# LPMP/BDD

Measured on AMD Instinct MI355X. Metric: parallel-MMA iterations/sec, 10.5M BDD nodes, 1 GPU (+ achieved HBM GB/s in roofline), higher is better.
Workload: dtype f32

## Files before the change

### bdd_amd/capi.py

```python
from __future__ import annotations

import ctypes as C
import os
import subprocess

_HERE = os.path.dirname(os.path.abspath(__file__))
LIB_PATH = os.path.abspath(os.environ["BDDMMA_LIB"]) if os.environ.get("BDDMMA_LIB") else os.path.join(_HERE, "csrc", "libbdd_mma_hip.so")

OK = 0
F32, F64 = 0, 1
K_FORWARD_MM, K_BACKWARD_MM, K_FINISH_DELTA, K_OTHER, K_COUNT = 0, 1, 2, 3, 4


class Options(C.Structure):
    _fields_ = [("pack_width", C.c_uint32), ("wide_pack_width", C.c_uint32), ("deterministic", C.c_uint32),
                ("vars_per_bin", C.c_uint32), ("stage_cap", C.c_uint32), ("waves_per_block", C.c_uint32),
                ("keep_bdd_order", C.c_uint32), ("resident_sweeps", C.c_uint32), ("exchange_by_variable", C.c_uint32),
                ("variant_flags", C.c_uint32), ("pack_fill", C.c_uint32), ("pack_stagger", C.c_uint32)]


class LbfgsParams(C.Structure):
    _fields_ = [("history_size", C.c_int32), ("init_step_size", C.c_double), ("req_rel_lb_increase", C.c_double),
                ("step_size_decrease_factor", C.c_double), ("step_size_increase_factor", C.c_double)]

# ... 58 lines not shown
    "bddmma_min_marginals": (_I, [_V, _I, _V, _V, _V, _I]),
    "bddmma_min_marginal_diff": (_I, [_V, _V, _I]),
    "bddmma_bdds_solution": (_I, [_V, _I, _V, _I]),
    "bddmma_net_solver_costs": (_I, [_V, _V, _I]),
    "bddmma_make_dual_feasible": (_I, [_V, _V, _I]),
    "bddmma_gradient_step": (_I, [_V, _V, _D, _I]),
    "bddmma_lbfgs_create": (_I, [C.POINTER(_V), _V, C.POINTER(LbfgsParams)]),
    "bddmma_lbfgs_destroy": (None, [_V]),
    "bddmma_lbfgs_iteration": (_I, [_V]),
    "bddmma_lbfgs_update_costs": (_I, [_V, _V, _U64, _V, _U64, _I, _I]),
    "bddmma_lbfgs_flush": (_I, [_V]),
    "bddmma_lbfgs_get_state": (_I, [_V, C.POINTER(LbfgsState)]),
    "bddmma_perturb_primal_costs": (_I, [_V, _V, _D, C.c_uint32, C.c_uint32, C.POINTER(C.c_uint32), _V, _V, _V]),
    "bddmma_run_solver": (_I, [_V, _V, _U64, _D, _D, _D, _I, C.POINTER(RunResult)]),
    "bddmma_run_solver_host_loop": (_I, [_V, _V, _U64, _D, _D, _D, _I, C.POINTER(RunResult)]),
    "bddmma_incremental_mm_agreement_rounding": (_I, [_V, _V, _D, _D, _U64, _U64, C.c_uint32, _I, _V, C.POINTER(_I)]),
    "bddmma_save": (_I, [_V, C.c_char_p]),
    "bddmma_load": (_I, [C.POINTER(_V), _I, C.c_char_p]),
    "bddmma_synchronize": (_I, [_V]),
    "bddmma_set_profiling": (_I, [_V, _I]),
    "bddmma_get_profile": (_I, [_V, C.POINTER(Profile)]),
    "bddmma_time_iterations": (_I, [_V, _D, _U64, C.POINTER(_D)]),
    "bddmma_time_kernel": (_I, [_V, _I, _U64, C.POINTER(_D)]),
    "bddmma_device_bytes": (_U64, [_V]),
    "bddmma_device_allocated_bytes": (_U64, [_V]),
    "bddmma_layout_create": (_I, [C.POINTER(_V), _V, _V, _U64, C.POINTER(Options)]),
    "bddmma_layout_create_for_chip": (_I, [C.POINTER(_V), _V, _V, _U64, C.POINTER(Options), _I, C.c_uint32, C.c_uint32]),
    "bddmma_layout_destroy": (None, [_V]),
    "bddmma_layout_size": (_U64, [_V, _I]),
    "bddmma_layout_copy": (_I, [_V, _I, _V]),
    "bddmma_layout_res2_records": (_I, [_V, _I, _V, _V, _V]),
    "bddmma_layout_stream_records": (_I, [_V, _I, _V, _V, _V]),
    "bddmma_layout_layer_records": (_I, [_V, _I, _V, _V, _V]),
    "bddmma_layout_seg_exchange": (_I, [_V, _I, _I, _V, _V, _V, _V]),
}

_I64P, _U64P = C.POINTER(C.c_int64), C.POINTER(C.c_uint64)
ILP_SIGNATURES = {
    "bddilp_last_error": (C.c_char_p, []),
    "bddilp_parse_lp": (_I, [C.c_char_p, C.POINTER(_V)]),
    "bddilp_parse_opb": (_I, [C.c_char_p, C.POINTER(_V)]),
    "bddilp_parse": (_I, [C.c_char_p, C.POINTER(_V)]),
    "bddilp_destroy": (None, [_V]),
    "bddilp_nr_variables": (_U64, [_V]),
    "bddilp_nr_constraints": (_U64, [_V]),
    "bddilp_variable_name": (C.c_char_p, [_V, _U64]),
    "bddilp_objective": (_I, [_V, _V, C.POINTER(_D)]),
    "bddilp_constraint_size": (_U64, [_V, _U64]),
    "bddilp_constraint": (_I, [_V, _U64, _V, _V, C.POINTER(_I), C.POINTER(C.c_int64)]),
    "bddilp_constraint_name": (C.c_char_p, [_V, _U64]),
    "bddilp_normalize": (_I, [_V]),
    "bddilp_to_bdds": (_I, [_V, _I, _U64, C.POINTER(_V)]),
    "bddilp_bdds_create": (_I, [C.POINTER(_V)]),
    "bddilp_bdds_add_row": (_I, [_V, _V, _V, _U64, _I, C.c_int64, C.POINTER(_I)]),
    "bddilp_bdds_split": (_I, [_V, _U64, _U64, _I, _U64P, _U64P]),
    "bddilp_bdds_destroy": (None, [_V]),
    "bddilp_bdds_nr_bdds": (_U64, [_V]),
    "bddilp_bdds_nr_instructions": (_U64, [_V]),
    "bddilp_bdds_nr_variables": (_U64, [_V]),
    "bddilp_bdds_instructions": (_V, [_V]),
    "bddilp_bdds_delimiters": (_V, [_V]),
    "bddilp_write_bdd_lp": (_I, [_V, _V, _U64, _V, _U64, C.c_char_p]),
    "bddilp_export_graphviz": (_I, [_V, _V, _U64, _U64, C.c_char_p]),
    "bddilp_random_set_cover": (_I, [_U64, _U64, _U64, _U64, _V, _V]),
}

# ... 35 lines not shown
```

### bdd_amd/csrc/capi.cpp

```cpp
#include <chrono>
#include <cmath>
#include <cstdio>
#include <cstdlib>
#include <cstring>
#include <limits>
#include <new>
#include <string>
#include <vector>

#include "../../include/bdd_mma.h"
#include "layout.hpp"
#include "solver.hpp"

using namespace bddmma;

struct bddmma_lbfgs;
extern "C" int bddmma_lbfgs_iteration(bddmma_lbfgs* l);
extern "C" int bddmma_lbfgs_update_costs(bddmma_lbfgs* l, const void* lo, uint64_t n_lo, const void* hi, uint64_t n_hi, int elem_precision,
                                         int on_device);

namespace {
thread_local std::string g_err;

template <typename F>
// ... 779 lines not shown
    if (!l || !info || (real_size != 4 && real_size != 8) || threads <= 0) return BDDMMA_ERR_INVALID_ARGUMENT;
    SegExchange S;
    build_seg_exchange(l->L, (uint32_t)threads, (uint32_t)real_size, S);
    info[0] = S.ok ? 1u : 0u; info[1] = (uint32_t)S.bin.size(); info[2] = (uint32_t)S.perm.size(); info[3] = (uint32_t)S.thr.size();
    info[4] = S.max_entries; info[5] = S.max_slots; info[6] = S.max_groups;
    if (bin && !S.bin.empty()) std::memcpy(bin, S.bin.data(), S.bin.size() * sizeof(uint32_t));
    if (perm && !S.perm.empty()) std::memcpy(perm, S.perm.data(), S.perm.size() * sizeof(uint16_t));
    if (thr && !S.thr.empty()) std::memcpy(thr, S.thr.data(), S.thr.size() * sizeof(uint32_t));
    return BDDMMA_OK;
}

int bddmma_layout_stream_records(const bddmma_layout* l, int real_size, uint32_t* info, uint32_t* words, uint32_t* rec_off)
{
    if (!l || !info || (real_size != 4 && real_size != 8)) return BDDMMA_ERR_INVALID_ARGUMENT;
    StreamRecords R;
    build_stream_records(l->L, (uint32_t)real_size, R);
    info[0] = R.ok ? 1u : 0u; info[1] = (uint32_t)R.rec.size();
    if (words && !R.rec.empty()) std::memcpy(words, R.rec.data(), R.rec.size() * sizeof(uint32_t));
    if (rec_off && !R.rec_off.empty()) std::memcpy(rec_off, R.rec_off.data(), R.rec_off.size() * sizeof(uint32_t));
    return BDDMMA_OK;
}

int bddmma_layout_layer_records(const bddmma_layout* l, int real_size, uint32_t* info, uint32_t* words, uint32_t* rec_off)
{
    if (!l || !info || (real_size != 4 && real_size != 8)) return BDDMMA_ERR_INVALID_ARGUMENT;
    LayerRecords R;
    build_layer_records(l->L, (uint32_t)real_size, R);
    info[0] = R.ok ? 1u : 0u; info[1] = (uint32_t)R.rec.size();
    if (words && !R.rec.empty()) std::memcpy(words, R.rec.data(), R.rec.size() * sizeof(uint32_t));
    if (rec_off && !R.rec_off.empty()) std::memcpy(rec_off, R.rec_off.data(), R.rec_off.size() * sizeof(uint32_t));
    return BDDMMA_OK;
}

}
```

### bdd_amd/csrc/kernels/narrow3.hpp

```cpp
#pragma once

namespace bddmma {

constexpr int N3_W = 128;
template <typename REAL>
__device__ __forceinline__ void lds_ld2(REAL& a, REAL& b, const unsigned char* lds, uint32_t off)
{
    const REAL* p = reinterpret_cast<const REAL*>(lds + off);
    a = p[0];
    b = p[1];
}

template <typename REAL, bool NT>
__device__ __forceinline__ void pot_pair_load(typename Pair<REAL>::type& v, rsrc_t rh, uint32_t voff, uint32_t soff)
{
    constexpr int AUX = NT ? 2 : BDDMMA_LD_POT_AUX;
    if constexpr (sizeof(REAL) == 4) v = __builtin_bit_cast(float2, __builtin_amdgcn_raw_buffer_load_b64(rh, voff, soff, AUX));
    else v = __builtin_bit_cast(double2, __builtin_amdgcn_raw_buffer_load_b128(rh, voff, soff, AUX));
}

__device__ __forceinline__ void pot_store(float v, rsrc_t rh, uint32_t voff, uint32_t soff, uint32_t ) { hop_store(v, rh, voff, soff); }
__device__ __forceinline__ void pot_store(double v, rsrc_t rh, uint32_t voff, uint32_t soff, uint32_t nt)
{
    if (nt) hop_store<2>(v, rh, voff, soff);
    else hop_store<>(v, rh, voff, soff);
}

template <typename REAL>
__device__ __forceinline__ void pot_store_layer(REAL a, REAL b, bool two, rsrc_t rh, uint32_t off_a, uint32_t soff, uint32_t nt)
{
    using P2 = typename Pair<REAL>::type;
    const uint32_t off2 = two ? off_a : (uint32_t)LREC_NO_STORE, off1 = two ? (uint32_t)LREC_NO_STORE : off_a;
    P2 v;
    v.x = a;
    v.y = b;
    if constexpr (sizeof(REAL) == 4) {
        using u2 = decltype(__builtin_amdgcn_raw_buffer_load_b64(rh, 0, 0, 0));
        __builtin_amdgcn_raw_buffer_store_b64(__builtin_bit_cast(u2, v), rh, off2, soff, BDDMMA_ST_FT_AUX_F32);
        pot_store(a, rh, off1, soff, nt);
    } else {
        using u4 = decltype(__builtin_amdgcn_raw_buffer_load_b128(rh, 0, 0, 0));
        const u4 data = __builtin_bit_cast(u4, v);
        if (nt) __builtin_amdgcn_raw_buffer_store_b128(data, rh, off2, soff, 2);
// ... 28 lines not shown
    const uint32_t quad = block_to_pack(block_id, n_quads, pk.xcd_chunk);
    BDDMMA_EXIT_IF(quad >= n_quads, d)
    const uint32_t p = quad * WPB + wave;
    const bool has_pack = p < pk.n_packs;
    const bool hdr = pk.hdr_pack != nullptr;
    const uint32_t* const hp = hdr ? pk.hdr_pack + 8 * (size_t)(has_pack ? p : 0) : nullptr;
    const uint32_t q0 = !has_pack ? 0 : (hdr ? hp[4] : pk.pack_hop_ptr[p]);
    const uint32_t q1 = !has_pack ? 0 : (hdr ? q0 + (hp[5] & 0xFFFFu) : pk.pack_hop_ptr[p + 1]);
    const uint32_t rbase = has_pack ? lrec_off[p] : 0;
    const uint32_t c0_h = hdr ? pk.hdr_quad[4 * (size_t)quad] : 0, cnt_h = hdr ? pk.hdr_quad[4 * (size_t)quad + 1] : 0;
    BDDMMA_STAMP(p, 0);
    const REAL INF = inf_v<REAL>();
    const uint32_t slot_first = !has_pack ? 0 : (hdr ? hp[0] : pk.hop_node_off[q0]), l0 = !has_pack ? 0 : (hdr ? hp[2] : pk.hop_layer_off[q0]);
    NarrowRs<REAL> rs(d);
    rs.rebase_layers(d, l0);
    uint32_t ent[STAGE_ITERS], esl[STAGE_ITERS];
    if (hdr) stage_load_tables<REAL, WPB, (NT ? 2 : BDDMMA_LD_TAB_AUX)>(ent, esl, rs, c0_h, cnt_h, tid);
    REAL* const Tp = d.T + slot_first;
    REAL* const Fp = d.F + slot_first;
    const REAL* const lohi_p = d.lohi + 2 * (size_t)l0;
    const rsrc_t rr = make_rsrc(lrec, lrec_words);
    HopWindow hw{sOffN_[wave], sOffL_[wave], sOffR_[wave], q0, q1, slot_first, l0};
    constexpr int D = LA;
    uint32_t o[2 * D + 3];
    uint32_t lb[D + 2];
    u4v rc[2 * D + 1];
    P2 tr[D + 1];
    P2 Lr[D + 1];
#pragma unroll
    for (int i = 0; i < 2 * D + 3; ++i) o[i] = 0;
#pragma unroll
    for (int i = 0; i < D + 2; ++i) lb[i] = 0;
    auto ldrec = [&](uint32_t h) { return __builtin_amdgcn_raw_buffer_load_b128(rr, (uint32_t)lane * 16u, (rbase + h * 64u) * 16u, 0); };
    const uint32_t sink = (W + 2 * (uint32_t)lane) * S;
    if (has_pack) {
        hw.fill(pk, q0, lane);
#pragma unroll
        for (int i = 0; i < 2 * D + 3; ++i) o[i] = hw.node_off(q0 + i);
#pragma unroll
        for (int i = 0; i < D + 2; ++i) lb[i] = hw.layer_off(q0 + i);
#pragma unroll
        for (int r = 0; r < 2; ++r) {
            const uint32_t j = lane + 64 * r;
            lds_st<REAL>(sFw, j * S, (j < o[1] - o[0]) ? REAL(0) : INF);
        }
#pragma unroll
        for (int b = 0; b < 2; ++b) {
            lds_st<REAL>(sTw, b * BUF + sink, REAL(0));
            lds_st<REAL>(sTw, b * BUF + sink + S, INF);
        }
#pragma unroll
        for (int i = 0; i < 2 * D; ++i) rc[i] = ldrec((uint32_t)i);
        {
            P2 t1;
            pot_pair_load<REAL, NT>(t1, hop_rsrc(Tp, o[1], o[2] - o[1]), 2u * (uint32_t)lane * S, o[1] * S);
#pragma unroll
            for (int i = 0; i < D; ++i) pot_pair_load<REAL, NT>(tr[i], hop_rsrc(Tp, o[i + 2], o[i + 3] - o[i + 2]), 2u * (uint32_t)lane * S, o[i + 2] * S);
            if (2u * (uint32_t)lane < o[2] - o[1]) lds_st<P2>(sTw, 2u * (uint32_t)lane * S, t1);
        }
#pragma unroll
        for (int i = 0; i < D; ++i) hop_load(Lr[i], rs.lohi, (uint32_t)lane * (uint32_t)sizeof(P2), lb[i] * (uint32_t)sizeof(P2));
        wave_sync();
    } else {
#pragma unroll
        for (int i = 0; i < 2 * D; ++i) rc[i] = u4v{0u, 0u, 0u, 0u};
    }
    uint32_t cur = 0;
    uint32_t q = q0;
    const uint32_t g0 = (has_pack && !hdr) ? pk.pack_group_ptr[p] : 0;
    const uint32_t ng = !has_pack ? 0 : (hdr ? 1u : pk.pack_group_ptr[p + 1] - g0);
    const uint32_t r0 = hdr ? 0 : pk.quad_round_ptr[quad];
    const uint32_t n_rounds = hdr ? 1u : pk.quad_round_ptr[quad + 1] - r0;
    const uint32_t db = (uint32_t)wave * pk.stage_cap * (uint32_t)sizeof(P2);
    for (uint32_t k = 0; k < n_rounds; ++k) {
    uint32_t gl0 = 0, cnt = 0, qe = q1;
    if (hdr) {
        cnt = cnt_h;
        stage_load_pairs<REAL, WPB>(sD, ent, esl, rs, cnt, tid);
        qe = has_pack ? q1 : q;
    } else {
        const uint32_t c0 = pk.cs_ptr[r0 + k];
        cnt = pk.cs_ptr[r0 + k + 1] - c0;
        stage_load<REAL, WPB, (NT ? 2 : BDDMMA_LD_TAB_AUX)>(sD, ent, esl, rs, c0, cnt, tid);
        if (k < ng) {
            gl0 = pk.grp_layer_off[g0 + k] - l0;
            qe = pk.grp_hop_end[g0 + k];
        } else {
            qe = q;
        }
    }
    if (WPB > 1) __syncthreads(); else wave_sync();
    BDDMMA_STAMP(p, 1);
    auto hop = [&]() {
        if (q + 2 * D + 3 >= hw.base + HOP_WIN && hw.base + HOP_WIN <= q1) hw.fill(pk, q, lane);
        const uint32_t nb = o[0];
        const uint32_t n3 = o[3] - o[2];
        const uint32_t fc = cur * BUF, fn = (cur ^ 1u) * BUF;
        const uint32_t stg = db + (lb[0] - gl0 + (uint32_t)lane) * (uint32_t)sizeof(P2);
        rc[2 * D] = ldrec(q - q0 + 2 * D);
#ifndef BDDMMA_EXP_NO_HOP_LOADS
        pot_pair_load<REAL, NT>(tr[D], hop_rsrc(Tp, o[D + 2], o[D + 3] - o[D + 2]), 2u * (uint32_t)lane * S, o[D + 2] * S);
        hop_load(Lr[D], rs.lohi, (uint32_t)lane * (uint32_t)sizeof(P2), lb[D] * (uint32_t)sizeof(P2));
#endif
        const u4v ra = rc[0];
        const P2 c = Lr[0];
        const uint32_t flags = ra[2] >> 16;
        REAL fa, fb;
        lds_ld2(fa, fb, sFw, fc + (ra[2] & 0xFFFFu));
        const REAL tla = lds_ld<REAL>(sTw, fc + (ra[0] & 0xFFFFu)), tha = lds_ld<REAL>(sTw, fc + (ra[0] >> 16));
        const REAL tlb = lds_ld<REAL>(sTw, fc + (ra[1] & 0xFFFFu)), thb = lds_ld<REAL>(sTw, fc + (ra[1] >> 16));
        const P2 dd = lds_ld<P2>(dyn_lds, stg);
        const uint32_t o_new = hw.node_off(q + 2 * D + 3);
        const uint32_t l_next = hw.layer_off(q + D + 2);
        if (2u * (uint32_t)lane < n3) lds_st<P2>(sTw, fn + 2u * (uint32_t)lane * S, tr[0]);
        lds_st<P2>(sFw, fn + 2u * (uint32_t)lane * S, P2{INF, INF});
        wave_sync();
        fa = (flags & LREC_REAL) ? fa : INF;
        fb = (flags & LREC_TWO) ? fb : INF;
        const REAL m0 = rmin((fa + c.x) + tla, (fb + c.x) + tlb);
        const REAL m1 = rmin((fa + c.y) + tha, (fb + c.y) + thb);
        const REAL mm = mm_diff1(m0, m1, omega);
        P2 nc;
        nc.x = (c.x + min0(mm)) + dd.x;
        nc.y = (c.y + min0_neg(mm)) + dd.y;
#ifndef BDDMMA_EXP_NO_HOP_STORES
        const rsrc_t rl = hop_rsrc(reinterpret_cast<const P2*>(lohi_p), lb[0], lb[1] - lb[0]);
        hop_store(nc, rl, (uint32_t)lane * (uint32_t)sizeof(P2), lb[0] * (uint32_t)sizeof(P2));
#endif
        if (flags & LREC_REAL) lds_st<REAL>(dyn_lds, stg, mm);
        lds_min(reinterpret_cast<REAL*>(sFw + fn + (ra[0] & 0xFFFFu)), fa + nc.x);
        lds_min(reinterpret_cast<REAL*>(sFw + fn + (ra[0] >> 16)), fa + nc.y);
        lds_min(reinterpret_cast<REAL*>(sFw + fn + (ra[1] & 0xFFFFu)), fb + nc.x);
        lds_min(reinterpret_cast<REAL*>(sFw + fn + (ra[1] >> 16)), fb + nc.y);
#ifndef BDDMMA_EXP_NO_HOP_STORES
        {
            const rsrc_t rf = hop_rsrc(Fp, nb, o[1] - o[0]);
            pot_store_layer<REAL>(fa, fb, (flags & LREC_TWO) != 0, rf, ra[3] & 0xFFFFu, nb * S, pk.nt_potentials);
        }
#endif
        wave_sync();
        cur ^= 1u;
#pragma unroll
        for (int i = 0; i < 2 * D + 2; ++i) o[i] = o[i + 1];
        o[2 * D + 2] = o_new;
#pragma unroll
        for (int i = 0; i < D + 1; ++i) lb[i] = lb[i + 1];
        lb[D + 1] = l_next;
#pragma unroll
// ... 55 lines not shown
    const uint32_t q0 = !has_pack ? 0 : (hdr ? hp[4] : pk.pack_hop_ptr[p]);
    const uint32_t q1 = !has_pack ? 0 : (hdr ? q0 + (hp[5] & 0xFFFFu) : pk.pack_hop_ptr[p + 1]);
    const uint32_t rbase = has_pack ? lrec_off[p] : 0;
    const uint32_t c0_h = hdr ? pk.hdr_quad[4 * (size_t)quad] : 0, cnt_h = hdr ? pk.hdr_quad[4 * (size_t)quad + 1] : 0;
    BDDMMA_STAMP(p, 0);
    const REAL INF = inf_v<REAL>();
    const uint32_t slot_first = !has_pack ? 0 : (hdr ? hp[0] : pk.hop_node_off[q0]), l0 = !has_pack ? 0 : (hdr ? hp[2] : pk.hop_layer_off[q0]);
    NarrowRs<REAL> rs(d);
    rs.rebase_layers(d, l0);
    uint32_t ent[STAGE_ITERS], esl[STAGE_ITERS];
    if (hdr) stage_load_tables<REAL, WPB, (NT ? 2 : BDDMMA_LD_TAB_AUX)>(ent, esl, rs, c0_h, cnt_h, tid);
    REAL* const Tp = d.T + slot_first;
    REAL* const Fp = d.F + slot_first;
    const REAL* const lohi_p = d.lohi + 2 * (size_t)l0;
    REAL* const x_p = d.x_layer != nullptr ? d.x_layer + l0 : nullptr;
    const rsrc_t rr = make_rsrc(lrec, lrec_words);
    HopWindow hw{sOffN_[wave], sOffL_[wave], sOffR_[wave], q0, q1, slot_first, l0};
    auto nb_of = [&](uint32_t qq) { return hw.node_off(qq); };
    constexpr int D = LA;
    uint32_t o[2 * D + 2];
    uint32_t lb[D + 2];
    u4v rc[2 * D + 1];
    P2 fr[D + 1];
    P2 Lr[D + 1];
#pragma unroll
    for (int i = 0; i < 2 * D + 2; ++i) o[i] = 0;
#pragma unroll
    for (int i = 0; i < D + 2; ++i) lb[i] = 0;
    uint32_t q = q1;
    auto ldrec = [&](uint32_t qq) { return __builtin_amdgcn_raw_buffer_load_b128(rr, (uint32_t)lane * 16u, (rbase + (qq >= q0 ? qq - q0 : 0u) * 64u) * 16u, 0); };
    auto ldf = [&](P2& f, const u4v& r, uint32_t nb, uint32_t n) {
        pot_pair_load<REAL, NT>(f, hop_rsrc(Fp, nb, n), r[3] & 0xFFFFu, nb * S);
    };
    const uint32_t sink = (W + 2 * (uint32_t)lane) * S;
    if (has_pack) {
#pragma unroll
        for (int b = 0; b < 2; ++b) {
            lds_st<REAL>(sTw, b * BUF + sink, REAL(0));
            lds_st<REAL>(sTw, b * BUF + sink + S, INF);
        }
        hw.fill(pk, q1 + 1 > q0 + HOP_WIN ? q1 + 1 - HOP_WIN : q0, lane);
#pragma unroll
        for (int i = 0; i < 2 * D + 2; ++i) o[i] = nb_of(q1 >= q0 + i ? q1 - i : q0);
#pragma unroll
        for (int i = 0; i < D + 2; ++i) lb[i] = hw.layer_off(q1 >= q0 + i ? q1 - i : q0);
#pragma unroll
        for (int i = 0; i < 2 * D; ++i) rc[i] = ldrec(q1 >= q0 + i + 1 ? q1 - 1 - i : q0);
#pragma unroll
        for (int i = 0; i < D; ++i) {
            ldf(fr[i], rc[i], o[i + 1], o[i] - o[i + 1]);
            hop_load(Lr[i], rs.lohi, (uint32_t)lane * (uint32_t)sizeof(P2), lb[i + 1] * (uint32_t)sizeof(P2));
        }
    } else {
#pragma unroll
        for (int i = 0; i < 2 * D; ++i) rc[i] = u4v{0u, 0u, 0u, 0u};
    }
    uint32_t cur = 0;
    const uint32_t g0 = (has_pack && !hdr) ? pk.pack_group_ptr[p] : 0;
    const uint32_t ng = !has_pack ? 0 : (hdr ? 1u : pk.pack_group_ptr[p + 1] - g0);
    const uint32_t r0 = hdr ? 0 : pk.quad_round_ptr[quad];
    const uint32_t n_rounds = hdr ? 1u : pk.quad_round_ptr[quad + 1] - r0;
    const uint32_t db = (uint32_t)wave * pk.stage_cap * (uint32_t)sizeof(P2);
    for (uint32_t k = n_rounds; k-- > 0;) {
    uint32_t gl0 = 0, cnt = 0, qs = q0;
    if (hdr) {
        cnt = cnt_h;
        stage_load_pairs<REAL, WPB>(sD, ent, esl, rs, cnt, tid);
        qs = has_pack ? q0 : q;
    } else {
        const uint32_t c0 = pk.cs_ptr[r0 + k];
        cnt = pk.cs_ptr[r0 + k + 1] - c0;
        stage_load<REAL, WPB, (NT ? 2 : BDDMMA_LD_TAB_AUX)>(sD, ent, esl, rs, c0, cnt, tid);
// ... 13 lines not shown
        const uint32_t tc = cur * BUF, tn = (cur ^ 1u) * BUF;
        const uint32_t stg = db + (lb[1] - gl0 + (uint32_t)lane) * (uint32_t)sizeof(P2);
        rc[2 * D] = ldrec(q >= q0 + 2 * D ? q - 2 * D : q0);
#ifndef BDDMMA_EXP_NO_HOP_LOADS
        ldf(fr[D], rc[D], o[D + 1], o[D] - o[D + 1]);
        hop_load(Lr[D], rs.lohi, (uint32_t)lane * (uint32_t)sizeof(P2), lb[D + 1] * (uint32_t)sizeof(P2));
#endif
        const u4v ra = rc[0];
        const P2 c = Lr[0];
        const uint32_t flags = ra[2] >> 16;
        const REAL tla = lds_ld<REAL>(sTw, tc + (ra[0] & 0xFFFFu)), tha = lds_ld<REAL>(sTw, tc + (ra[0] >> 16));
        const REAL tlb = lds_ld<REAL>(sTw, tc + (ra[1] & 0xFFFFu)), thb = lds_ld<REAL>(sTw, tc + (ra[1] >> 16));
        const P2 dd = lds_ld<P2>(dyn_lds, stg);
        const uint32_t o_new = (q >= q0 + 2 * D + 1) ? nb_of(q - 1 - 2 * D) : o[2 * D + 1];
        const uint32_t l_next = hw.layer_off(q >= q0 + D + 1 ? q - 1 - D : q0);
        const REAL fa = (flags & LREC_REAL) ? fr[0].x : INF;
        const REAL fb = (flags & LREC_TWO) ? fr[0].y : INF;
        const REAL m0 = rmin((fa + c.x) + tla, (fb + c.x) + tlb);
        const REAL m1 = rmin((fa + c.y) + tha, (fb + c.y) + thb);
        const REAL mm = mm_diff1(m0, m1, omega);
        P2 nc;
        nc.x = (c.x + min0(mm)) + dd.x;
        nc.y = (c.y + min0_neg(mm)) + dd.y;
        const REAL ta = rmin(nc.y + tha, nc.x + tla);
        const REAL tb = rmin(nc.y + thb, nc.x + tlb);
#ifndef BDDMMA_EXP_NO_HOP_STORES
        const rsrc_t rl = hop_rsrc(reinterpret_cast<const P2*>(lohi_p), lb[1], lb[0] - lb[1]);
        hop_store(nc, rl, (uint32_t)lane * (uint32_t)sizeof(P2), lb[1] * (uint32_t)sizeof(P2));
#endif
        if (flags & LREC_REAL) {
            lds_st<REAL>(dyn_lds, stg, mm);
            lds_st<REAL>(sTw, tn + (ra[2] & 0xFFFFu), ta);
        }
        if (flags & LREC_TWO) lds_st<REAL>(sTw, tn + (ra[2] & 0xFFFFu) + S, tb);
        if (x_p != nullptr) {
            const rsrc_t rx = hop_rsrc(x_p, lb[1], lb[0] - lb[1]);
            hop_store((nc.y - nc.x) + mm, rx, (uint32_t)lane * S, lb[1] * S);
        }
#ifndef BDDMMA_EXP_NO_HOP_STORES
        {
            const rsrc_t rt = hop_rsrc(Tp, nb, o[0] - o[1]);
            pot_store_layer<REAL>(ta, tb, (flags & LREC_TWO) != 0, rt, ra[3] & 0xFFFFu, nb * S, pk.nt_potentials);
        }
#endif
        wave_sync();
        cur ^= 1u;
#pragma unroll
        for (int i = 0; i < 2 * D + 1; ++i) o[i] = o[i + 1];
        o[2 * D + 1] = o_new;
#pragma unroll
        for (int i = 0; i < D + 1; ++i) lb[i] = lb[i + 1];
        lb[D + 1] = l_next;
#pragma unroll
        for (int i = 0; i < 2 * D; ++i) rc[i] = rc[i + 1];
#pragma unroll
        for (int i = 0; i < D; ++i) {
            Lr[i] = Lr[i + 1];
            fr[i] = fr[i + 1];
        }
    };
    while (q >= qs + HOP_UNROLL) {
#pragma unroll
        for (int u = 0; u < HOP_UNROLL; ++u) hop();
    }
    while (q > qs) hop();
    BDDMMA_STAMP(p, 3);
    if (WPB > 1) __syncthreads(); else wave_sync();
    BDDMMA_STAMP(p, 2);
    stage_flush<REAL, WPB>(sD, ent, esl, rs, cnt, tid);
    BDDMMA_STAMP(p, 4);
    if (WPB > 1 && k > 0) __syncthreads();
    }
    if (!has_pack) return;
    const uint32_t n0 = nb_of(q0 + 1) - nb_of(q0);
    double s = 0.0;
#pragma unroll
    for (int r = 0; r < 2; ++r) {
        const uint32_t j = lane + 64 * r;
        if (j < n0) s += (double)lds_ld<REAL>(sTw, cur * BUF + j * S);
    }
    for (int off2 = 32; off2 > 0; off2 >>= 1) s += __shfl_down(s, off2);
    if (lane == 0) d.lb_partial[pk.lb_base + p] = s;
}

template <typename REAL, int WPB, bool NT = false>
__global__ void __launch_bounds__(64 * WPB) __attribute__((amdgpu_waves_per_eu(BDDMMA_N3_WAVES(REAL)))) k_bwd_narrow3(DevPtrs<REAL> d, PackDev pk, const uint32_t* __restrict__ lrec, const uint32_t* __restrict__ lrec_off,
                                                          uint32_t lrec_words, REAL omega)
{
    bwd_narrow3_body<REAL, WPB, NT, BDDMMA_N3_LOOKAHEAD(REAL)>(d, pk, lrec, lrec_off, lrec_words, omega, blockIdx.x);
}

}
```

### bdd_amd/csrc/layout.cpp

```cpp
#include "layout.hpp"

#include <algorithm>
#include <atomic>
#include <chrono>
#include <cstdio>
#include <cstdlib>
#include <mutex>
#include <thread>
#include <unordered_map>
#include <cstring>
#include <limits>

namespace bddmma {

namespace {

std::atomic<unsigned> g_layout_threads{0};
thread_local unsigned t_layout_threads = 0;
struct Par {
    unsigned nt = 1;
    Par()
    {
        const char* e = std::getenv("BDDMMA_THREADS");
        const unsigned hw = std::thread::hardware_concurrency();
// ... 1184 lines not shown
            for (uint32_t l = 0; l < 64; ++l) {
                const uint32_t bot = (W + 2 * l + 1) * S;
                r[4 * l + 0] = r[4 * l + 1] = bot | (bot << 16);
                r[4 * l + 2] = (W + 2 * l) * S;
                r[4 * l + 3] = LREC_NO_STORE | (LREC_NO_STORE << 16);
            }
            uint32_t l = 0;
            for (uint32_t j = 0; j < n; ++j) {
                const uint32_t w = words[nb + j];
                if (w & NW_PAD) continue;
                const uint32_t pos = (w >> NW_POS_SHIFT) & NW_FIELD6;
                const uint32_t lo = w & NW_CHILD_MASK, hi = (w >> NW_CHILD_BITS) & NW_CHILD_MASK;
                auto child = [&](uint32_t c, uint32_t lane) { return (c < W ? c : W + 2 * lane + (c - W)) * S; };
                if (pos == 0) {
                    if (l >= nl) { out = LayerRecords(); return; }
                    r[4 * l + 0] = child(lo, l) | (child(hi, l) << 16);
                    r[4 * l + 2] = (j * S) | (LREC_REAL << 16);
                    r[4 * l + 3] = (j * S) | (LREC_NO_STORE << 16);
                    ++l;
                } else {
                    if (pos != 1 || l == 0 || !(w & NW_TWO) || (r[4 * (l - 1) + 2] & 0xFFFFu) != (j - 1) * S) { out = LayerRecords(); return; }
                    const uint32_t k = l - 1;
                    r[4 * k + 1] = child(lo, k) | (child(hi, k) << 16);
                    r[4 * k + 2] |= LREC_TWO << 16;
                    r[4 * k + 3] = (r[4 * k + 3] & 0xFFFFu) | ((j * S) << 16);
                }
            }
            if (l != nl) { out = LayerRecords(); return; }
        }
    }
    out.ok = true;
}

void set_layout_threads(unsigned n) { g_layout_threads.store(n, std::memory_order_relaxed); }
void set_thread_layout_threads(unsigned n) { t_layout_threads = n; }

}
```

### bdd_amd/csrc/layout.hpp

```cpp
#pragma once
#include <cstdint>
#include <string>
#include <vector>

#include "../../include/bdd_mma.h"

#ifndef __host__
#define __host__
#define __device__
#endif

namespace bddmma {

constexpr uint32_t NW_CHILD_BITS = 9;
constexpr uint32_t NW_CHILD_MASK = (1u << NW_CHILD_BITS) - 1;
constexpr uint32_t NW_POS_SHIFT = 18, NW_LIDX_SHIFT = 24, NW_FIELD6 = 63;
constexpr uint32_t NW_TWO = 1u << 30;
constexpr uint32_t NW_PAD = 1u << 31;
constexpr uint32_t nw_top(uint32_t pack_width) { return pack_width; }
constexpr uint32_t nw_bot(uint32_t pack_width) { return pack_width + 1; }
constexpr uint32_t nw_pad_word(uint32_t pack_width)
{
    return NW_PAD | (nw_bot(pack_width) << NW_CHILD_BITS) | nw_bot(pack_width);
}
// ... 119 lines not shown
constexpr uint32_t RES2_NO_STORE = 0xFFF0u;
constexpr uint32_t RES2_PAD = 0xFFFFFFFFu;
struct Res2Records {
    bool ok = false;
    std::vector<uint32_t> rec;
    std::vector<uint32_t> rec_off;
    uint32_t max_hops = 0;
};
__host__ __device__ inline uint32_t res2_t_off() { return 0; }
__host__ __device__ inline uint32_t res2_f_off(uint32_t real_size, uint32_t ns) { return (ns + 4u) * real_size; }
__host__ __device__ inline uint32_t res2_c_off(uint32_t real_size, uint32_t ns) { return (ns + 4u) * real_size + (ns + 64u) * real_size; }
__host__ __device__ inline uint32_t res2_wave_bytes(uint32_t real_size, uint32_t ns, uint32_t nl) { return res2_c_off(real_size, ns) + nl * 2u * real_size; }
inline uint32_t res2_slot_capacity(uint32_t real_size, uint32_t max_slots) { const uint32_t q = 1024u / real_size; return (max_slots + q - 1) / q * q; }
inline uint32_t res2_layer_capacity(uint32_t real_size, uint32_t max_layers) { const uint32_t q = 512u / real_size; return (max_layers + q - 1) / q * q; }
void build_res2_records(const HostLayout& L, uint32_t real_size, uint32_t ns, uint32_t nl, Res2Records& out);

constexpr uint32_t SREC_PAD = 0x80000000u;
struct StreamRecords {
    bool ok = false;
    std::vector<uint32_t> rec;
    std::vector<uint32_t> rec_off;
};
void build_stream_records(const HostLayout& L, uint32_t real_size, StreamRecords& out);

constexpr uint32_t LREC_NO_STORE = 0xFFF0u;
constexpr uint32_t LREC_TWO = 1u, LREC_REAL = 2u;
struct LayerRecords {
    bool ok = false;
    std::vector<uint32_t> rec;
    std::vector<uint32_t> rec_off;
};
void build_layer_records(const HostLayout& L, uint32_t real_size, LayerRecords& out);

struct LinComb {
    const char* g;
    const void* S;
    const char* Y;
    uint64_t slot;
    const double* cy;
    const double* cs;
    const uint32_t* order;
    int ns;
};
constexpr int LINCOMB_MAX = 8;

struct SegExchange {
    bool ok = false;
    uint32_t threads = 0;
    uint32_t max_entries = 0, max_slots = 0, max_groups = 0;
    std::vector<uint32_t> bin;
    std::vector<uint16_t> perm;
    std::vector<uint32_t> thr;
};
constexpr uint32_t SEG_MAX_RUN = 32;
void build_seg_exchange(const HostLayout& L, uint32_t threads, uint32_t real_size, SegExchange& out);

struct ChipInfo {
    uint32_t n_cus = 256;
    uint32_t lds_bytes = 160 * 1024;
    uint64_t max_resident_threads = 256ull * 2048;
};

int build_layout(const bddmma_instruction* instr, const uint64_t* delims, uint64_t n_bdds,
                 const bddmma_options* opts, HostLayout& out, std::string& err, bool keep_debug_maps,
                 uint32_t real_size = 4, ChipInfo chip = ChipInfo{});

// ... 2 lines not shown
```

### bdd_amd/csrc/solver_impl.hpp

```cpp
#pragma once
#include <hip/hip_runtime.h>
#include <atomic>
#include <chrono>
#include <cmath>
#include <cstdio>
#include <cstdlib>
#include <cstring>
#include <limits>
#include <memory>
#include <string>
#include <thread>
#include <vector>
#include "../../include/bdd_mma.h"
#include "kernels.hpp"
#include "layout.hpp"
#include "solver.hpp"

namespace bddmma {

static inline void cpu_relax()
{
#if defined(__x86_64__) || defined(__i386__)
    __asm__ __volatile__("pause");
#elif defined(__aarch64__)
// ... 441 lines not shown
                    case 64: SET_RES_W(1) break;
                    case 128: SET_RES_W(2) break;
                    default: SET_RES_W(4) break;
                }
#undef SET_RES_W
#undef SET_RES
            }
        }
        uint32_t narrow2_static = 0;
        if (nb_.n_packs && !use_res && !wb_.n_packs && !(opts && (opts->variant_flags & 0x1000u))) {
            StreamRecords SR;
            build_stream_records(L, sizeof(REAL), SR);
            narrow2_static = L.ex.waves_per_block * ((2 * pack_width + 2 + pack_width + 2) * (uint32_t)sizeof(REAL) + 3 * 64 * 4 + 64);
            const bool forced = opts && (opts->variant_flags & 0x2000u);
            const bool shared = forced || (SR.rec.size() * sizeof(uint32_t) <= (uint64_t)L.narrow_slots * sizeof(REAL) / 2 &&
                                           (sizeof(REAL) == 8 || n_slots <= 16'000'000ull));
            if (SR.ok && shared && stage_lds + narrow2_static + seg_bytes(L.ex.waves_per_block) <= 64 * 1024) {
                if ((rc = upload(&d_srec, SR.rec))) return rc;
                if ((rc = upload(&d_srec_off, SR.rec_off))) return rc;
                srec_words = (uint32_t)SR.rec.size();
                use_narrow2 = true;
                narrow_gen = narrow_seg;
                for (uint16_t r : L.narrow.hop_root) narrow_gen = narrow_gen || r != NO_ROOT;
            }
        }
        if (nb_.n_packs && !use_res && !wb_.n_packs && !hb_.n_packs && !narrow_seg && pack_width == 128 && (L.ex.waves_per_block == 4 || L.ex.waves_per_block == 8) &&
            !(opts && (opts->variant_flags & 0x41000u))) {
            LayerRecords LR;
            build_layer_records(L, sizeof(REAL), LR);
            const uint32_t n3_static = L.ex.waves_per_block * (4 * (128 + 128) * (uint32_t)sizeof(REAL) + 3 * 64 * 4);
            const bool forced = opts && (opts->variant_flags & 0x2000u);
            const bool shared = forced || (LR.rec.size() * sizeof(uint32_t) <= (uint64_t)L.narrow_slots * sizeof(REAL) / 2 && n_slots <= 16'000'000ull);
            if (LR.ok && shared && stage_lds + n3_static <= lds_cu - 1024) {
                if ((rc = upload(&d_lrec, LR.rec))) return rc;
                if ((rc = upload(&d_lrec_off, LR.rec_off))) return rc;
                lrec_words = (uint32_t)LR.rec.size();
                use_narrow3 = true;
                n3_nt = sizeof(REAL) == 8 && nt_potentials != 0;
#define SET_N3(W_, NT_)                                                                                                                              \
    HIPCHK(hipFuncSetAttribute(reinterpret_cast<const void*>(&k_fwd_narrow3<REAL, W_, NT_>), hipFuncAttributeMaxDynamicSharedMemorySize, (int)stage_lds)); \
    HIPCHK(hipFuncSetAttribute(reinterpret_cast<const void*>(&k_bwd_narrow3<REAL, W_, NT_>), hipFuncAttributeMaxDynamicSharedMemorySize, (int)stage_lds));
                if (L.ex.waves_per_block == 4) { SET_N3(4, false) } else { SET_N3(8, false) }
                if constexpr (sizeof(REAL) == 8) {
                    if (L.ex.waves_per_block == 4) { SET_N3(4, true) } else { SET_N3(8, true) }
                }
#undef SET_N3
            }
        }
        if (nb_.n_packs && !use_res && !use_narrow3 && !wb_.n_packs && !hb_.n_packs && !narrow_seg && !narrow_gen && pack_width == 128 &&
            (L.ex.waves_per_block == 4 || L.ex.waves_per_block == 8) && (beyond_cache || (opts && (opts->variant_flags & 0x100000u))))
#ifndef BDDMMA_EXP_NO_N12_NT
            n12_nt = !use_narrow2 || sizeof(REAL) == 8;
#else
            n12_nt = false;
#endif
        nt_loads = n3_nt || n12_nt;
        if (wb_.n_packs) {
            wide_threads = std::min<uint32_t>(1024, std::max<uint32_t>(64, ((wide_pack_width + 1) / 2 + 63) / 64 * 64));
            wide_npt = (wide_pack_width + wide_threads - 1) / wide_threads;
            wide_npt = wide_npt <= 1 ? 1 : (wide_npt <= 2 ? 2 : 4);
            wide_lds = (uint32_t)wide2_lds_bytes(sizeof(REAL), wide_pack_width, true);
            if (wide_lds > lds_cu || wide_pack_width > 4096) {
                err = "wide_pack_width " + std::to_string(wide_pack_width) + " needs " + std::to_string(wide_lds) + " B of LDS (> 160 KiB)";
                return BDDMMA_ERR_UNSUPPORTED;
            }
#define SET_LDS(K) HIPCHK(hipFuncSetAttribute(reinterpret_cast<const void*>(&K), hipFuncAttributeMaxDynamicSharedMemorySize, (int)wide_lds))
// ... 1124 lines not shown
```

### include/bdd_mma.h

```cpp
#ifndef BDD_MMA_H
#define BDD_MMA_H

#include <stddef.h>
#include <stdint.h>

#ifdef __cplusplus
extern "C" {
#endif

#define BDDMMA_OK 0
#define BDDMMA_ERR_INVALID_ARGUMENT (-1)
#define BDDMMA_ERR_INVALID_BDD (-2)
#define BDDMMA_ERR_DEVICE (-3)
#define BDDMMA_ERR_STATE (-4)
#define BDDMMA_ERR_UNSUPPORTED (-5)
#define BDDMMA_ERR_IO (-6)

#define BDDMMA_F32 0
#define BDDMMA_F64 1

typedef struct bddmma_instruction {
    uint64_t lo;
    uint64_t hi;
    uint64_t index;
// ... 133 lines not shown

int bddmma_save(const bddmma_solver* s, const char* path);
int bddmma_load(bddmma_solver** out, int device, const char* path);

int bddmma_synchronize(bddmma_solver* s);
#define BDDMMA_K_FORWARD_MM 0
#define BDDMMA_K_BACKWARD_MM 1
#define BDDMMA_K_FINISH_DELTA 2
#define BDDMMA_K_OTHER 3
#define BDDMMA_K_COUNT 4
typedef struct bddmma_profile {
    uint64_t launches[BDDMMA_K_COUNT];
    double total_ms[BDDMMA_K_COUNT];
} bddmma_profile;
int bddmma_set_profiling(bddmma_solver* s, int on);
int bddmma_get_profile(bddmma_solver* s, bddmma_profile* out);
int bddmma_time_iterations(bddmma_solver* s, double omega, uint64_t n, double* ms);
#define BDDMMA_TRIAD_BYTES (1ull << 30)
int bddmma_time_kernel(bddmma_solver* s, int kind, uint64_t reps, double* ms);
uint64_t bddmma_device_bytes(const bddmma_solver* s);
uint64_t bddmma_device_allocated_bytes(const bddmma_solver* s);

typedef struct bddmma_layout bddmma_layout;
int bddmma_layout_create(bddmma_layout** out, const bddmma_instruction* instr, const uint64_t* bdd_delims,
                         uint64_t n_bdds, const bddmma_options* opts);
int bddmma_layout_create_for_chip(bddmma_layout** out, const bddmma_instruction* instr, const uint64_t* bdd_delims,
                                  uint64_t n_bdds, const bddmma_options* opts, int real_size, uint32_t n_cus, uint32_t lds_bytes_per_cu);
void bddmma_layout_destroy(bddmma_layout* l);
uint64_t bddmma_layout_size(const bddmma_layout* l, int what);
int bddmma_layout_copy(const bddmma_layout* l, int which, void* out);
int bddmma_layout_res2_records(const bddmma_layout* l, int real_size, uint32_t* info, uint32_t* words, uint32_t* rec_off);
int bddmma_layout_stream_records(const bddmma_layout* l, int real_size, uint32_t* info, uint32_t* words, uint32_t* rec_off);
int bddmma_layout_layer_records(const bddmma_layout* l, int real_size, uint32_t* info, uint32_t* words, uint32_t* rec_off);
int bddmma_layout_seg_exchange(const bddmma_layout* l, int threads, int real_size, uint32_t* info, uint32_t* bin, uint16_t* perm, uint32_t* thr);

#ifdef __cplusplus
}
#endif
#endif
```

Measured before the change: 8775.

## Remap narrow-kernel LDS hop slots to split pair halves and avoid bank conflicts

Introduces an LDS slot permutation for the narrow3 kernel's hop buffers: even node indices go to the first 128 slots and odd ones to a second, rotated half-bank. Layer records are rewritten on the host to carry mapped offsets, including an explicit second-node offset in a spare field. Pair stores and loads become two scalar accesses at separated addresses. The aim is to reduce LDS bank conflicts on the strided pair accesses. In exchange there are more LDS instructions, a host-side validation pass, and the risk of rejecting layouts whose offsets fall outside 256 entries.

```diff
diff --git a/bdd_amd/capi.py b/bdd_amd/capi.py
--- a/bdd_amd/capi.py
+++ b/bdd_amd/capi.py
@@ -114,6 +114,7 @@
     "bddmma_layout_res2_records": (_I, [_V, _I, _V, _V, _V]),
     "bddmma_layout_stream_records": (_I, [_V, _I, _V, _V, _V]),
     "bddmma_layout_layer_records": (_I, [_V, _I, _V, _V, _V]),
+    "bddmma_layer_records_lds_map": (_I, [_V, _U64, _I]),
     "bddmma_layout_seg_exchange": (_I, [_V, _I, _I, _V, _V, _V, _V]),
 }
 
diff --git a/bdd_amd/csrc/capi.cpp b/bdd_amd/csrc/capi.cpp
--- a/bdd_amd/csrc/capi.cpp
+++ b/bdd_amd/csrc/capi.cpp
@@ -835,4 +835,10 @@
     return BDDMMA_OK;
 }
 
-}
+int bddmma_layer_records_lds_map(uint32_t* words, uint64_t n_words, int real_size)
+{
+    if ((n_words && !words) || (real_size != 4 && real_size != 8)) return BDDMMA_ERR_INVALID_ARGUMENT;
+    return layer_records_lds_map(words, (size_t)n_words, (uint32_t)real_size) ? BDDMMA_OK : BDDMMA_ERR_INVALID_ARGUMENT;
+}
+
+}
diff --git a/bdd_amd/csrc/kernels/narrow3.hpp b/bdd_amd/csrc/kernels/narrow3.hpp
--- a/bdd_amd/csrc/kernels/narrow3.hpp
+++ b/bdd_amd/csrc/kernels/narrow3.hpp
@@ -3,12 +3,14 @@
 namespace bddmma {
 
 constexpr int N3_W = 128;
-template <typename REAL>
-__device__ __forceinline__ void lds_ld2(REAL& a, REAL& b, const unsigned char* lds, uint32_t off)
-{
-    const REAL* p = reinterpret_cast<const REAL*>(lds + off);
-    a = p[0];
-    b = p[1];
+static_assert(N3_W == 128, "n3_lds_slot maps hop buffers of 128 slots + 128 sinks");
+template <typename P2>
+__device__ __forceinline__ void lds_st_pair(unsigned char* lds, uint32_t off, P2 v)
+{
+    using REAL = decltype(v.x);
+    REAL* p = reinterpret_cast<REAL*>(lds + off);
+    p[0] = v.x;
+    p[N3_PAIR_B] = v.y;
 }
 
 template <typename REAL, bool NT>
@@ -103,7 +105,8 @@
 #pragma unroll
     for (int i = 0; i < D + 2; ++i) lb[i] = 0;
     auto ldrec = [&](uint32_t h) { return __builtin_amdgcn_raw_buffer_load_b128(rr, (uint32_t)lane * 16u, (rbase + h * 64u) * 16u, 0); };
-    const uint32_t sink = (W + 2 * (uint32_t)lane) * S;
+    const uint32_t top = n3_lds_slot(W + 2 * (uint32_t)lane) * S, bot = n3_lds_slot(W + 2 * (uint32_t)lane + 1) * S;
+    const uint32_t pair = (uint32_t)lane * S;
     if (has_pack) {
         hw.fill(pk, q0, lane);
 #pragma unroll
@@ -113,12 +116,12 @@
 #pragma unroll
         for (int r = 0; r < 2; ++r) {
             const uint32_t j = lane + 64 * r;
-            lds_st<REAL>(sFw, j * S, (j < o[1] - o[0]) ? REAL(0) : INF);
+            lds_st<REAL>(sFw, n3_lds_slot(j) * S, (j < o[1] - o[0]) ? REAL(0) : INF);
         }
 #pragma unroll
         for (int b = 0; b < 2; ++b) {
-            lds_st<REAL>(sTw, b * BUF + sink, REAL(0));
-            lds_st<REAL>(sTw, b * BUF + sink + S, INF);
+            lds_st<REAL>(sTw, b * BUF + top, REAL(0));
+            lds_st<REAL>(sTw, b * BUF + bot, INF);
         }
 #pragma unroll
         for (int i = 0; i < 2 * D; ++i) rc[i] = ldrec((uint32_t)i);
@@ -127,7 +130,7 @@
             pot_pair_load<REAL, NT>(t1, hop_rsrc(Tp, o[1], o[2] - o[1]), 2u * (uint32_t)lane * S, o[1] * S);
 #pragma unroll
             for (int i = 0; i < D; ++i) pot_pair_load<REAL, NT>(tr[i], hop_rsrc(Tp, o[i + 2], o[i + 3] - o[i + 2]), 2u * (uint32_t)lane * S, o[i + 2] * S);
-            if (2u * (uint32_t)lane < o[2] - o[1]) lds_st<P2>(sTw, 2u * (uint32_t)lane * S, t1);
+            if (2u * (uint32_t)lane < o[2] - o[1]) lds_st_pair(sTw, pair, t1);
         }
 #pragma unroll
         for (int i = 0; i < D; ++i) hop_load(Lr[i], rs.lohi, (uint32_t)lane * (uint32_t)sizeof(P2), lb[i] * (uint32_t)sizeof(P2));
@@ -176,15 +179,14 @@
         const u4v ra = rc[0];
         const P2 c = Lr[0];
         const uint32_t flags = ra[2] >> 16;
-        REAL fa, fb;
-        lds_ld2(fa, fb, sFw, fc + (ra[2] & 0xFFFFu));
+        REAL fa = lds_ld<REAL>(sFw, fc + (ra[2] & 0xFFFFu)), fb = lds_ld<REAL>(sFw, fc + (ra[3] >> 16));
         const REAL tla = lds_ld<REAL>(sTw, fc + (ra[0] & 0xFFFFu)), tha = lds_ld<REAL>(sTw, fc + (ra[0] >> 16));
         const REAL tlb = lds_ld<REAL>(sTw, fc + (ra[1] & 0xFFFFu)), thb = lds_ld<REAL>(sTw, fc + (ra[1] >> 16));
         const P2 dd = lds_ld<P2>(dyn_lds, stg);
         const uint32_t o_new = hw.node_off(q + 2 * D + 3);
         const uint32_t l_next = hw.layer_off(q + D + 2);
-        if (2u * (uint32_t)lane < n3) lds_st<P2>(sTw, fn + 2u * (uint32_t)lane * S, tr[0]);
-        lds_st<P2>(sFw, fn + 2u * (uint32_t)lane * S, P2{INF, INF});
+        if (2u * (uint32_t)lane < n3) lds_st_pair(sTw, fn + pair, tr[0]);
+        lds_st_pair(sFw, fn + pair, P2{INF, INF});
         wave_sync();
         fa = (flags & LREC_REAL) ? fa : INF;
         fb = (flags & LREC_TWO) ? fb : INF;
@@ -306,12 +308,12 @@
     auto ldf = [&](P2& f, const u4v& r, uint32_t nb, uint32_t n) {
         pot_pair_load<REAL, NT>(f, hop_rsrc(Fp, nb, n), r[3] & 0xFFFFu, nb * S);
     };
-    const uint32_t sink = (W + 2 * (uint32_t)lane) * S;
+    const uint32_t top = n3_lds_slot(W + 2 * (uint32_t)lane) * S, bot = n3_lds_slot(W + 2 * (uint32_t)lane + 1) * S;
     if (has_pack) {
 #pragma unroll
         for (int b = 0; b < 2; ++b) {
-            lds_st<REAL>(sTw, b * BUF + sink, REAL(0));
-            lds_st<REAL>(sTw, b * BUF + sink + S, INF);
+            lds_st<REAL>(sTw, b * BUF + top, REAL(0));
+            lds_st<REAL>(sTw, b * BUF + bot, INF);
         }
         hw.fill(pk, q1 + 1 > q0 + HOP_WIN ? q1 + 1 - HOP_WIN : q0, lane);
 #pragma unroll
@@ -391,7 +393,7 @@
             lds_st<REAL>(dyn_lds, stg, mm);
             lds_st<REAL>(sTw, tn + (ra[2] & 0xFFFFu), ta);
         }
-        if (flags & LREC_TWO) lds_st<REAL>(sTw, tn + (ra[2] & 0xFFFFu) + S, tb);
+        if (flags & LREC_TWO) lds_st<REAL>(sTw, tn + (ra[3] >> 16), tb);
         if (x_p != nullptr) {
             const rsrc_t rx = hop_rsrc(x_p, lb[1], lb[0] - lb[1]);
             hop_store((nc.y - nc.x) + mm, rx, (uint32_t)lane * S, lb[1] * S);
@@ -436,7 +438,7 @@
 #pragma unroll
     for (int r = 0; r < 2; ++r) {
         const uint32_t j = lane + 64 * r;
-        if (j < n0) s += (double)lds_ld<REAL>(sTw, cur * BUF + j * S);
+        if (j < n0) s += (double)lds_ld<REAL>(sTw, cur * BUF + n3_lds_slot(j) * S);
     }
     for (int off2 = 32; off2 > 0; off2 >>= 1) s += __shfl_down(s, off2);
     if (lane == 0) d.lb_partial[pk.lb_base + p] = s;
diff --git a/bdd_amd/csrc/layout.cpp b/bdd_amd/csrc/layout.cpp
--- a/bdd_amd/csrc/layout.cpp
+++ b/bdd_amd/csrc/layout.cpp
@@ -1240,6 +1240,31 @@
     out.ok = true;
 }
 
+bool layer_records_lds_map(uint32_t* rec, size_t n_words, uint32_t S)
+{
+    if ((S != 4 && S != 8) || n_words % 4 != 0 || (n_words && !rec)) return false;
+    const uint32_t n_ent = 256;
+    auto entry_ok = [&](uint32_t off) { return off % S == 0 && off / S < n_ent; };
+    for (size_t i = 0; i < n_words; i += 4) {
+        const uint32_t* r = rec + i;
+        const uint32_t flags = r[2] >> 16;
+        if (!entry_ok(r[0] & 0xFFFFu) || !entry_ok(r[0] >> 16) || !entry_ok(r[1] & 0xFFFFu) || !entry_ok(r[1] >> 16) || !entry_ok(r[2] & 0xFFFFu))
+            return false;
+        if ((flags & LREC_TWO) && (r[2] & 0xFFFFu) / S + 1 >= 128) return false;
+    }
+    auto map = [&](uint32_t off) { return n3_lds_slot(off / S) * S; };
+    for (size_t i = 0; i < n_words; i += 4) {
+        uint32_t* r = rec + i;
+        const uint32_t own = r[2] & 0xFFFFu, flags = r[2] >> 16, lane = (uint32_t)(i / 4 % 64);
+        const uint32_t second = (flags & LREC_TWO) ? map(own + S) : n3_lds_slot(128u + 2u * lane + 1u) * S;
+        r[0] = map(r[0] & 0xFFFFu) | (map(r[0] >> 16) << 16);
+        r[1] = map(r[1] & 0xFFFFu) | (map(r[1] >> 16) << 16);
+        r[2] = map(own) | (flags << 16);
+        r[3] = (r[3] & 0xFFFFu) | (second << 16);
+    }
+    return true;
+}
+
 void set_layout_threads(unsigned n) { g_layout_threads.store(n, std::memory_order_relaxed); }
 void set_thread_layout_threads(unsigned n) { t_layout_threads = n; }
 
diff --git a/bdd_amd/csrc/layout.hpp b/bdd_amd/csrc/layout.hpp
--- a/bdd_amd/csrc/layout.hpp
+++ b/bdd_amd/csrc/layout.hpp
@@ -175,6 +175,10 @@
 };
 void build_layer_records(const HostLayout& L, uint32_t real_size, LayerRecords& out);
 
+constexpr uint32_t N3_PAIR_B = 128u + 16u;
+constexpr uint32_t n3_lds_slot(uint32_t j) { return (j & 1u) ? 128u + (((j >> 1) + 16u) & 127u) : (j >> 1); }
+bool layer_records_lds_map(uint32_t* rec, size_t n_words, uint32_t real_size);
+
 struct LinComb {
     const char* g;
     const void* S;
diff --git a/bdd_amd/csrc/solver_impl.hpp b/bdd_amd/csrc/solver_impl.hpp
--- a/bdd_amd/csrc/solver_impl.hpp
+++ b/bdd_amd/csrc/solver_impl.hpp
@@ -497,6 +497,7 @@
             const bool forced = opts && (opts->variant_flags & 0x2000u);
             const bool shared = forced || (LR.rec.size() * sizeof(uint32_t) <= (uint64_t)L.narrow_slots * sizeof(REAL) / 2 && n_slots <= 16'000'000ull);
             if (LR.ok && shared && stage_lds + n3_static <= lds_cu - 1024) {
+                if (!layer_records_lds_map(LR.rec.data(), LR.rec.size(), sizeof(REAL))) { err = "layer records: an offset outside a hop buffer"; return BDDMMA_ERR_INVALID_ARGUMENT; }
                 if ((rc = upload(&d_lrec, LR.rec))) return rc;
                 if ((rc = upload(&d_lrec_off, LR.rec_off))) return rc;
                 lrec_words = (uint32_t)LR.rec.size();
diff --git a/include/bdd_mma.h b/include/bdd_mma.h
--- a/include/bdd_mma.h
+++ b/include/bdd_mma.h
@@ -189,6 +189,7 @@
 int bddmma_layout_res2_records(const bddmma_layout* l, int real_size, uint32_t* info, uint32_t* words, uint32_t* rec_off);
 int bddmma_layout_stream_records(const bddmma_layout* l, int real_size, uint32_t* info, uint32_t* words, uint32_t* rec_off);
 int bddmma_layout_layer_records(const bddmma_layout* l, int real_size, uint32_t* info, uint32_t* words, uint32_t* rec_off);
+int bddmma_layer_records_lds_map(uint32_t* words, uint64_t n_words, int real_size);
 int bddmma_layout_seg_exchange(const bddmma_layout* l, int threads, int real_size, uint32_t* info, uint32_t* bin, uint16_t* perm, uint32_t* thr);
 
 #ifdef __cplusplus
```

Result: no change. 8786, median of 6 (+0.1%).
